# SilasK/drep

Measured on AMD Instinct MI355X. Metric: genome pairs/sec (mash dist, k=21 s=1000) + sketch GB/s, at 1/2/4/8 GPUs, higher is better.
Workload: dtype u64; 1 GPU; 1000 synthetic 5000000 bp genomes, k=21, s=1000 (BASELINE.json configs[1]); step = sketch + all-pairs (one GPU: no all-gather); genomes=1000, genome_bp=5000000, k=21, sketch=1000, family_size=100, parallelism=sketch: genome shards; all-pairs: balanced row shards; RCCL all-gather

## Files before the change

drep_amd/_lib.py:

```python
from __future__ import annotations

import ctypes as C
import importlib.util
import os
import sys
import threading
from typing import Optional, Sequence, Tuple

import numpy as np

_HERE = os.path.dirname(os.path.abspath(__file__))
LIB_PATH = os.environ.get("DREPHIP_LIB", os.path.join(_HERE, "lib", "libdrephip.so"))

ERR = {0: "OK", -1: "invalid argument", -2: "HIP error", -3: "I/O error", -4: "out of memory",
       -5: "unsupported", -6: "internal error"}


class DrepHipError(RuntimeError):
    pass


_lib = None
_lock = threading.Lock()

u64p = np.ctypeslib.ndpointer(dtype=np.uint64, flags="C_CONTIGUOUS")
u32p = np.ctypeslib.ndpointer(dtype=np.uint32, flags="C_CONTIGUOUS")
u16p = np.ctypeslib.ndpointer(dtype=np.uint16, flags="C_CONTIGUOUS")
u8p = np.ctypeslib.ndpointer(dtype=np.uint8, flags="C_CONTIGUOUS")
f64p = np.ctypeslib.ndpointer(dtype=np.float64, flags="C_CONTIGUOUS")
vp = C.c_void_p

SIGNATURES = {
    "drephip_version": (C.c_int, []),
    "drephip_build_id": (C.c_char_p, []),
    "drephip_last_error": (C.c_char_p, []),
    "drephip_device_count": (C.c_int, [C.POINTER(C.c_int)]),
    "drephip_create": (C.c_int, [C.c_int, C.c_int, C.c_uint32, C.c_uint32, C.POINTER(vp)]),
    "drephip_destroy": (C.c_int, [vp]),
    "drephip_max_sketch": (C.c_uint32, []),
    "drephip_tile_bases": (C.c_uint64, []),
    "drephip_padded_bases": (C.c_uint64, [u64p, C.c_uint32]),
    "drephip_fasta_info": (C.c_int, [C.c_char_p, C.c_int, C.POINTER(C.c_uint64), C.POINTER(C.c_uint64),
                                     C.POINTER(C.c_uint32), C.POINTER(C.c_uint64)]),
    "drephip_fasta_pack": (C.c_int, [C.c_char_p, C.c_int, u32p, u32p, C.c_uint64, C.c_uint64,
                                     C.POINTER(C.c_uint64), C.POINTER(C.c_uint64)]),
    "drephip_sketch": (C.c_int, [vp, u8p, u64p, C.c_uint32, u64p, C.c_uint32, u64p, u32p, u64p]),
    "drephip_sketch_files": (C.c_int, [vp, C.POINTER(C.c_char_p), C.c_uint32, C.c_int, u64p, u32p, u64p]),
    "drephip_last_ingest_stats": (C.c_int, [vp, C.POINTER(C.c_double), C.POINTER(C.c_double),
                                            C.POINTER(C.c_double), C.POINTER(C.c_uint32)]),
    "drephip_last_ingest_phases": (C.c_int, [vp, C.POINTER(C.c_double), C.POINTER(C.c_double),
                                             C.POINTER(C.c_uint32)]),
    "drephip_sketch_device": (C.c_int, [vp, vp, vp, u64p, u64p, u64p, C.c_uint32, vp, vp, vp]),
    "drephip_sketch_device_async": (C.c_int, [vp, vp, vp, u64p, u64p, u64p, C.c_uint32, vp, vp, vp]),
    "drephip_sketch_wait": (C.c_int, [vp, C.POINTER(C.c_int)]),
    "drephip_synth_device": (C.c_int, [vp, C.c_uint64, C.c_uint32, C.c_uint32, C.c_uint32, C.c_uint64,
                                       vp, vp, vp]),
    "drephip_prefilter_eval": (C.c_int, [u64p, u64p, C.c_uint64, C.c_uint64, u8p, u8p]),
    "drephip_allpairs": (C.c_int, [vp, u64p, u32p, C.c_uint32, u16p, vp]),
    "drephip_allpairs_rows": (C.c_int, [vp, u64p, u32p, C.c_uint32, C.c_uint32, C.c_uint32, vp, vp]),
    "drephip_allpairs_device": (C.c_int, [vp, vp, vp, C.c_uint32, C.c_uint32, C.c_uint32, vp, vp, vp]),
    "drephip_allpairs_device_async": (C.c_int, [vp, vp, vp, C.c_uint32, C.c_uint32, C.c_uint32, vp, vp, vp]),
    "drephip_allpairs_wait": (C.c_int, [vp]),
    "drephip_screen_geometry": (C.c_int, [vp, C.POINTER(C.c_uint32)]),
    "drephip_screen_part": (C.c_int, [vp, vp, vp, C.c_uint32, C.c_uint32, C.c_uint32, C.POINTER(C.c_uint64),
                                      C.POINTER(C.c_uint32), C.POINTER(C.c_uint32), vp]),
    "drephip_screen_part_copy": (C.c_int, [vp, vp, vp, vp]),
    "drephip_screen_worth": (C.c_int, [vp, C.c_uint32, C.c_uint64, C.POINTER(C.c_int), C.POINTER(C.c_int)]),
    "drephip_allpairs_device_marked": (C.c_int, [vp, vp, vp, C.c_uint32, C.c_uint32, C.c_uint32, vp, vp, vp,
                                                 C.c_uint64, vp, C.c_uint64, vp]),
    "drephip_allpairs_merge_device": (C.c_int, [vp, vp, vp, C.c_uint32, C.c_uint32, C.c_uint32, vp, vp, vp]),
    "drephip_allpairs_sparse_device": (C.c_int, [vp, vp, vp, C.c_uint32, C.c_uint32, C.c_uint32, vp, C.c_uint64,
                                                 C.POINTER(C.c_uint64), vp]),
    "drephip_allpairs_sparse": (C.c_int, [vp, u64p, u32p, C.c_uint32, C.c_uint32, C.c_uint32, vp, C.c_uint64,
                                          C.POINTER(C.c_uint64)]),
    "drephip_last_sparse_stats": (C.c_int, [vp, C.POINTER(C.c_uint32), C.POINTER(C.c_uint64), C.POINTER(C.c_uint64),
                                            C.POINTER(C.c_uint64)]),
    "drephip_distance_lut": (C.c_int, [C.c_int, C.c_uint32, f64p]),
    "drephip_write_mash_table": (C.c_int, [C.c_char_p, C.POINTER(C.c_char_p), C.c_uint32, vp, vp, C.c_uint32,
                                           vp, vp, u16p, f64p, C.c_int]),
    "drephip_set_allpairs_path": (C.c_int, [vp, C.c_int, C.c_uint32]),
    "drephip_linkage": (C.c_int, [vp, f64p, C.c_uint32, C.c_int, f64p]),
    "drephip_linkage_counts_device": (C.c_int, [vp, vp, vp, C.c_uint32, u32p, f64p, C.c_uint32,
                                                np.ctypeslib.ndpointer(dtype=np.int32, flags="C_CONTIGUOUS"),
                                                C.c_int, f64p, vp]),
    "drephip_linkage_square": (C.c_int, [vp, np.ctypeslib.ndpointer(dtype=np.float32, flags="C_CONTIGUOUS"),
                                         C.c_uint32, C.c_int, f64p]),
    "drephip_mdb_square": (C.c_int, [C.c_uint32, vp, vp, C.c_uint32, vp, C.c_uint32, vp, vp, C.c_int, vp, vp, vp,
                                     vp, C.c_int]),
    "drephip_pivot_scan": (C.c_int, [C.c_uint64, vp, vp, C.c_int, C.c_uint32, u8p, u8p, C.POINTER(C.c_uint64),
                                     C.c_int]),
    "drephip_pivot_fill": (C.c_int, [C.c_uint64, vp, vp, C.c_int, vp, vp, C.c_uint32, vp, C.c_uint32, C.c_uint32,
                                     C.c_uint64, vp, C.c_int]),
    "drephip_linkage_reserve": (C.c_int, [vp, C.c_uint32]),
    "drephip_set_linkage_path": (C.c_int, [vp, C.c_int]),
    "drephip_linkage_sparse": (C.c_int, [C.c_uint32, C.c_uint64, u32p, u32p, f64p, C.c_int, f64p]),
    "drephip_last_linkage_info": (C.c_int, [vp, C.POINTER(C.c_int), C.POINTER(C.c_uint64), C.POINTER(C.c_uint32),
                                            C.POINTER(C.c_uint32)]),
    "drephip_last_linkage_stats": (C.c_int, [vp] + [C.POINTER(C.c_double)] * 5),
    "drephip_last_linkage_launches": (C.c_int, [vp, C.POINTER(C.c_uint64)]),
    "drephip_set_timing": (C.c_int, [vp, C.c_int]),
    "drephip_last_kernel_ms": (C.c_int, [vp, C.c_int, C.POINTER(C.c_double), C.POINTER(C.c_int)]),
    "drephip_set_allpairs_screen": (C.c_int, [vp, C.c_int]),
    "drephip_last_screen_stats": (C.c_int, [vp, C.POINTER(C.c_int), C.POINTER(C.c_uint64), C.POINTER(C.c_uint64),
                                             C.POINTER(C.c_uint64), C.POINTER(C.c_uint64), C.POINTER(C.c_uint64)]),
}


def _preload_torch_hip_runtime() -> None:
    if "torch" in sys.modules:
        return
# ... 52 lines not shown
    return hashlib.sha256(listing.encode()).hexdigest()


def build_id() -> dict:
    raw = lib().drephip_build_id().decode()
    return dict(kv.split("=", 1) for kv in raw.split(";") if "=" in kv)


def check(rc: int, what: str) -> None:
    if rc != 0:
        msg = lib().drephip_last_error().decode("utf-8", "replace")
        raise DrepHipError("%s failed (%s): %s" % (what, ERR.get(rc, rc), msg))


def device_count() -> int:
    n = C.c_int(0)
    rc = lib().drephip_device_count(C.byref(n))
    return n.value if rc == 0 else 0


def max_sketch() -> int:
    return int(lib().drephip_max_sketch())


def tile_bases() -> int:
    return int(lib().drephip_tile_bases())


def padded_bases(rec_len: Sequence[int]) -> int:
    a = np.ascontiguousarray(rec_len, dtype=np.uint64)
    return int(lib().drephip_padded_bases(a if len(a) else np.zeros(1, np.uint64), len(a)))


def distance_lut(denom: int, k: int = 21) -> np.ndarray:
    out = np.zeros(denom + 1, dtype=np.float64)
    check(lib().drephip_distance_lut(k, denom, out), "drephip_distance_lut")
    return out


def prefilter_eval(q1: np.ndarray, q2: np.ndarray, T: int) -> Tuple[np.ndarray, np.ndarray]:
    q1 = np.ascontiguousarray(q1, dtype=np.uint64)
    q2 = np.ascontiguousarray(q2, dtype=np.uint64)
    if q1.shape != q2.shape or q1.ndim != 1:
        raise ValueError("q1 and q2 must be equal-length vectors")
    n = len(q1)
    ok = np.zeros(max(n, 1), np.uint8)
    exact = np.zeros(max(n, 1), np.uint8)
    z = np.zeros(1, np.uint64)
    check(lib().drephip_prefilter_eval(q1 if n else z, q2 if n else z, n, int(T), ok, exact),
          "drephip_prefilter_eval")
    return ok[:n].astype(bool), exact[:n].astype(bool)


def write_mash_table(path: str, names: Sequence[str], common: np.ndarray, denom: Optional[np.ndarray], s: int,
                     dist: np.ndarray, pval: np.ndarray, self_count: np.ndarray, self_pval: np.ndarray,
                     threads: int = 0) -> None:
    N = len(names)
    npairs = N * (N - 1) // 2
    common = np.ascontiguousarray(common, dtype=np.uint16)
    dist = np.ascontiguousarray(dist, dtype=np.float64)
    pval = np.ascontiguousarray(pval, dtype=np.float64)
    for a in (common, dist, pval) + ((denom,) if denom is not None else ()):
        if len(a) != npairs:
            raise ValueError("condensed arrays must hold N(N-1)/2 = %d entries" % npairs)
    den = None if denom is None else np.ascontiguousarray(denom, dtype=np.uint16)
    arr = (C.c_char_p * max(N, 1))(*[os.fsencode(n) for n in names])
    check(lib().drephip_write_mash_table(os.fsencode(path), arr, N, common.ctypes.data,
                                         None if den is None else den.ctypes.data, int(s), dist.ctypes.data,
                                         pval.ctypes.data, np.ascontiguousarray(self_count, dtype=np.uint16),
                                         np.ascontiguousarray(self_pval, dtype=np.float64), int(threads)),
          "drephip_write_mash_table(%s)" % path)


def fasta_info(path: str, k: int = 21):
    length = C.c_uint64(0)
    padded = C.c_uint64(0)
    nrec = C.c_uint32(0)
    nk = C.c_uint64(0)
    check(lib().drephip_fasta_info(path.encode(), k, C.byref(length), C.byref(padded), C.byref(nrec),
                                   C.byref(nk)), "drephip_fasta_info(%s)" % path)
    return {"length": length.value, "padded": padded.value, "n_records": nrec.value, "n_kmers": nk.value}


def _ptr(a: Optional[np.ndarray]):
    return None if a is None else a.ctypes.data


def mdb_square(N: int, common: np.ndarray, denom: Optional[np.ndarray], s: int, lut32: np.ndarray,
               lut_off: np.ndarray, codes: np.ndarray, threads: int = 0, want_sim: bool = True):
    common = np.ascontiguousarray(common, dtype=np.uint16)
    den = None if denom is None else np.ascontiguousarray(denom, dtype=np.uint16)
    lut32 = np.ascontiguousarray(lut32, dtype=np.float32)
    lut_off = np.ascontiguousarray(lut_off, dtype=np.int32)
    codes = np.ascontiguousarray(codes)
    if codes.dtype not in (np.int8, np.int16, np.int32) or len(codes) != N or len(lut_off) != s + 1:
        raise ValueError("codes must be N int8/int16/int32 category codes and lut_off s+1 offsets")
    npairs = N * (N - 1) // 2
    if len(common) != npairs or (den is not None and len(den) != npairs):
        raise ValueError("condensed arrays must hold N(N-1)/2 = %d entries" % npairs)
    codes32 = codes.astype(np.int32)
    g1 = np.empty(N * N, dtype=codes.dtype)
    g2 = np.empty(N * N, dtype=codes.dtype)
    dist = np.empty(N * N, dtype=np.float32)
    sim = np.empty(N * N, dtype=np.float32) if want_sim else None
    check(lib().drephip_mdb_square(N, _ptr(common) if npairs else None, _ptr(den) if npairs else None, int(s),
                                   _ptr(lut32), len(lut32), _ptr(lut_off), _ptr(codes32), codes.dtype.itemsize,
# ... 376 lines not shown
```

drep_amd/csrc/api.cpp:

```cpp
#include "ctx.h"
#include "prefilter.h"
#include "../../include/drephip.h"

#include <algorithm>
#include <atomic>
#include <chrono>
#include <cmath>
#include <condition_variable>
#include <mutex>
#include <cstdlib>
#include <cstring>
#include <new>
#include <thread>
#include <vector>

#define DREPHIP_EXPORT extern "C" __attribute__((visibility("default")))

namespace drephip {

static thread_local std::string g_err;
void set_error(const std::string &msg) { g_err = msg; }

int scratch(drephip_ctx *ctx, const char *name, size_t bytes, void **out) {
    DevBuf &b = ctx->bufs[name];
    if (bytes == 0) bytes = 8;
    if (b.bytes < bytes) {
        const size_t want = std::max(bytes, b.bytes + b.bytes / 4);
        if (b.ptr) {
            HIPC(hipStreamSynchronize(ctx->stream));
            HIPC(hipDeviceSynchronize());
            HIPC(hipFree(b.ptr));
            b.ptr = nullptr; b.bytes = 0;
        }
        ctx->alloc_gen++;
        hipError_t e = hipMalloc(&b.ptr, want);
        if (e != hipSuccess) {
            set_error(std::string("hipMalloc(") + std::to_string(want) + ") for " + name + ": " +
                      hipGetErrorString(e));
            b.ptr = nullptr;
            return DREPHIP_ERR_NOMEM;
        }
        b.bytes = want;
    }
    *out = b.ptr;
    return DREPHIP_OK;
}

int pinned_host(drephip_ctx *ctx, const char *name, size_t bytes, void **out) {
    DevBuf &b = ctx->pinned[name];
    if (bytes == 0) bytes = 8;
    if (b.bytes < bytes) {
        if (b.ptr) {
            HIPC(hipStreamSynchronize(ctx->stream));
// ... 818 lines not shown
    int rc;
    if ((rc = scratch(ctx, "ap_in_h", (uint64_t)N * s * 8, (void **)&d_h))) return rc;
    if ((rc = scratch(ctx, "ap_in_n", N * 4ull, (void **)&d_n))) return rc;
    if (cap && (rc = scratch(ctx, "sp_out", cap * 16, (void **)&d_p))) return rc;
    HIPC(hipMemcpyAsync(d_h, hashes, (uint64_t)N * s * 8, hipMemcpyHostToDevice, st));
    HIPC(hipMemcpyAsync(d_n, nhash, N * 4ull, hipMemcpyHostToDevice, st));
    timing_begin(ctx);
    rc = allpairs_sparse_impl(ctx, d_h, d_n, N, row0, row1, (uint4 *)d_p, cap, n_pairs, st);
    if (rc && rc != DREPHIP_ERR_NOMEM) return rc;
    timing_collect(ctx);
    const uint64_t have = std::min(*n_pairs, cap);
    if (have) HIPC(hipMemcpyAsync(pairs, d_p, have * 16, hipMemcpyDeviceToHost, st));
    HIPC(hipStreamSynchronize(st));
    return rc;
}

DREPHIP_EXPORT int drephip_last_sparse_stats(drephip_ctx *ctx, uint32_t *blocks, uint64_t *direct, uint64_t *fallback,
                                             uint64_t *scratch_bytes) {
    if (!ctx) { set_error("null context"); return DREPHIP_ERR_ARG; }
    if (blocks) *blocks = ctx->sparse.blocks;
    if (direct) *direct = ctx->sparse.direct;
    if (fallback) *fallback = ctx->sparse.fallback;
    if (scratch_bytes) *scratch_bytes = ctx->sparse.scratch_bytes;
    return DREPHIP_OK;
}

DREPHIP_EXPORT int drephip_distance_lut(int k, uint32_t denom, double *lut) {
    if (!lut || k < 1 || denom == 0) { set_error("bad argument"); return DREPHIP_ERR_ARG; }
    for (uint32_t c = 0; c <= denom; c++) {
        double d;
        if (c == denom) d = 0.0;
        else if (c == 0) d = 1.0;
        else {
            const double j = (double)c / (double)denom;
            d = -std::log(2.0 * j / (1.0 + j)) / (double)k;
            if (d > 1.0) d = 1.0;
        }
        lut[c] = d;
    }
    return DREPHIP_OK;
}

DREPHIP_EXPORT int drephip_prefilter_eval(const uint64_t *q1, const uint64_t *q2, uint64_t n, uint64_t T,
                                          uint8_t *pass, uint8_t *exact) {
    if (n && (!q1 || !q2 || !pass || !exact)) { set_error("bad argument"); return DREPHIP_ERR_ARG; }
    const uint32_t Tp = prefilter_bound(T);
    for (uint64_t i = 0; i < n; i++) {
        pass[i] = prefilter_hi(q1[i], q2[i]) <= Tp;
        exact[i] = murmur_fin(q1[i], q2[i]) <= T;
    }
    return DREPHIP_OK;
}

constexpr uint64_t kSparseMaxCells = 1ull << 31;
constexpr uint64_t kSparseMaxPairs = 1ull << 26;

static uint64_t env_u64(const char *name, uint64_t dflt) {
    if (const char *e = std::getenv(name)) return std::strtoull(e, nullptr, 10);
    return dflt;
}
static uint64_t sparse_cells(const drephip_ctx *ctx) {
    return ctx->link_path == DREPHIP_LINK_PATH_SPARSE ? kSparseMaxCells : env_u64("DREPHIP_LINK_SPARSE_CELLS", 1ull << 28);
}
static uint32_t sparse_maxcomp(const drephip_ctx *ctx) {
    return ctx->link_path == DREPHIP_LINK_PATH_SPARSE ? 0xFFFFFFFFu
                                                      : (uint32_t)env_u64("DREPHIP_LINK_SPARSE_MAXCOMP", 4096);
}
static uint64_t sparse_pair_cap(const drephip_ctx *ctx, uint32_t n) {
    const uint64_t all = (uint64_t)n * (n - 1) / 2;
    const uint64_t cap = ctx->link_path == DREPHIP_LINK_PATH_SPARSE ? kSparseMaxPairs
                                                                    : std::min<uint64_t>(kSparseMaxPairs, 32ull * n + (1ull << 20));
    return std::min(all, cap);
}

DREPHIP_EXPORT int drephip_set_linkage_path(drephip_ctx *ctx, int path) {
    GUARD_CTX(ctx);
    if (path < DREPHIP_LINK_PATH_AUTO || path > DREPHIP_LINK_PATH_SPARSE) { set_error("bad linkage path"); return DREPHIP_ERR_ARG; }
    ctx->link_path = path;
    return DREPHIP_OK;
}

DREPHIP_EXPORT int drephip_linkage_sparse(uint32_t n, uint64_t npairs, const uint32_t *i, const uint32_t *j,
                                          const double *v, int method, double *Z) {
    if (n < 2) return DREPHIP_OK;
    if (!Z || (npairs && (!i || !j || !v))) { set_error("null argument"); return DREPHIP_ERR_ARG; }
    return linkage_sparse_impl(n, npairs, i, j, v, method, kSparseMaxCells, 0xFFFFFFFFu, Z, nullptr, 1);
}

static int linkage_condensed_sparse(drephip_ctx *ctx, const double *y, uint32_t n, int method, double *Z, int *rc) {
    *rc = DREPHIP_OK;
    if (ctx->link_path == DREPHIP_LINK_PATH_DENSE) return 0;
    const double t0 = std::chrono::duration<double>(std::chrono::steady_clock::now().time_since_epoch()).count();
    const uint64_t np_all = (uint64_t)n * (n - 1) / 2, cap = sparse_pair_cap(ctx, n);
    const unsigned T = host_threads();
    std::vector<uint32_t> rb(T + 1, n - 1);
    rb[0] = 0;
    for (unsigned k = 1; k < T; k++) {
        const uint64_t target = np_all * k / T;
        uint32_t lo = rb[k - 1], hi = n - 1;
        while (lo < hi) {
            const uint32_t mid = lo + (hi - lo) / 2;
            if ((uint64_t)mid * n - (uint64_t)mid * (mid + 1) / 2 < target) lo = mid + 1; else hi = mid;
        }
        rb[k] = lo;
    }
    std::vector<std::vector<uint32_t>> qi(T), qj(T);
// ... 208 lines not shown
```

drep_amd/csrc/prefilter.h:

```cpp
#pragma once

#include <hip/hip_runtime.h>
#include <stdint.h>

namespace drephip {

constexpr uint64_t kFmixC1 = 0xff51afd7ed558ccdULL;
constexpr uint64_t kFmixC2 = 0xc4ceb9fe1a85ec53ULL;

__host__ __device__ __forceinline__ uint32_t mulhi32(uint32_t a, uint32_t b) {
#if defined(__HIP_DEVICE_COMPILE__)
    return __umulhi(a, b);
#else
    return (uint32_t)(((uint64_t)a * b) >> 32);
#endif
}

__host__ __device__ __forceinline__ uint64_t fmix64_q(uint64_t k) {
    k ^= k >> 33; k *= kFmixC1;
    k ^= k >> 33;
    return k;
}
__host__ __device__ __forceinline__ uint64_t fmix_mul(uint64_t q) { return q * kFmixC2; }
__host__ __device__ __forceinline__ uint64_t murmur_fin(uint64_t q1, uint64_t q2) {
    const uint64_t p1 = fmix_mul(q1), p2 = fmix_mul(q2);
    return (p1 ^ (p1 >> 33)) + (p2 ^ (p2 >> 33));
}

__host__ __device__ __forceinline__ uint32_t prefilter_bound(uint64_t T) {
    return __builtin_elementwise_add_sat((uint32_t)(T >> 32), 2u);
}
__host__ __device__ __forceinline__ uint32_t prefilter_hi(uint64_t q1, uint64_t q2) {
    const uint64_t Q = q1 + q2;
    const uint32_t a = (uint32_t)Q, b = (uint32_t)(Q >> 32);
    return mulhi32(a, (uint32_t)kFmixC2) + a * (uint32_t)(kFmixC2 >> 32) + b * (uint32_t)kFmixC2 + 1u;
}

}
```

drep_amd/csrc/sketch.hip:

```cpp

#include "ctx.h"
#include "prefilter.h"
#include "../../include/drephip.h"

#include <algorithm>
#include <cstddef>
#include <cstdio>
#include <cstdlib>
#include <cstring>
#include <vector>

namespace drephip {

__device__ __forceinline__ void set_insert(unsigned long long *S, uint32_t mask, uint32_t *cnt,
                                           uint32_t limit, uint64_t h) {
    if (__hip_atomic_load(cnt, __ATOMIC_RELAXED, __HIP_MEMORY_SCOPE_AGENT) >= limit) return;
    uint32_t slot = (uint32_t)h & mask;
    for (uint32_t probe = 0; probe <= mask; probe++) {
        unsigned long long old = atomicCAS(&S[slot], (unsigned long long)kEmpty, (unsigned long long)h);
        if (old == kEmpty) { atomicAdd(cnt, 1u); return; }
        if (old == h) return;
        slot = (slot + 1) & mask;
    }
}

__device__ __forceinline__ uint64_t rotl64_ab(uint64_t x, int r) {
    const uint32_t lo = (uint32_t)x, hi = (uint32_t)(x >> 32);
    uint32_t nlo, nhi;
    if (r < 32) {
        nhi = __builtin_amdgcn_alignbit(hi, lo, 32 - r);
        nlo = __builtin_amdgcn_alignbit(lo, hi, 32 - r);
    } else {
        nhi = __builtin_amdgcn_alignbit(lo, hi, 64 - r);
        nlo = __builtin_amdgcn_alignbit(hi, lo, 64 - r);
    }
    return ((uint64_t)nhi << 32) | nlo;
}
__device__ __forceinline__ uint64_t x5_plus(uint64_t x, uint64_t c) {
    uint64_t y;
    asm("v_lshl_add_u64 %0, %1, 2, %1" : "=v"(y) : "v"(x));
    return y + c;
}
__device__ __forceinline__ uint64_t add64(uint64_t a, uint64_t b) {
    uint64_t y;
    asm("v_lshl_add_u64 %0, %1, 0, %2" : "=v"(y) : "v"(a), "v"(b));
    return y;
}
#ifndef DREPHIP_SK_STAGE
#define DREPHIP_SK_STAGE 128
#endif
constexpr uint32_t kStage = DREPHIP_SK_STAGE;

typedef uint32_t u32x4 __attribute__((ext_vector_type(4)));
typedef uint32_t u32x2 __attribute__((ext_vector_type(2)));
struct SketchTablesQ {
    u32x4 e1[256];
    u32x4 e2[256];
    u32x2 b1[256];
    u32x2 b2[256];
    uint64_t t3[1024];
};

__device__ __forceinline__ uint32_t ascii4(uint32_t x) {
    const uint32_t sel = ((x >> 6) & 3u) | (((x >> 4) & 3u) << 8) | (((x >> 2) & 3u) << 16) | ((x & 3u) << 24);
    return __builtin_amdgcn_perm(0u, 0x54474341u, sel);
}

__device__ void build_tables(SketchTablesQ &tb, uint32_t tid, uint32_t nthreads) {
    constexpr uint64_t c1 = 0x87c37b91114253d5ULL, c2 = 0x4cf5ad432745937fULL;
    for (uint32_t x = tid; x < 256; x += nthreads) {
        const uint32_t a = ascii4(x);
        const uint64_t A1 = (uint64_t)a * c1, A2 = (uint64_t)a * c2;
        const uint32_t x1 = (uint32_t)A1, x2 = (uint32_t)A2;
        const uint32_t ta1 = (uint32_t)(A1 >> 32), ta2 = (uint32_t)(A2 >> 32);
        const uint64_t t1 = ((uint64_t)x1 << 31) * c2 + ((uint64_t)(ta1 << 31) << 32);
        const uint64_t t2 = ((uint64_t)(x2 & 0x7fffffffu) << 33) * c1 + (uint64_t)(x2 >> 31) * c1;
        tb.e1[x] = u32x4{(uint32_t)t1, (uint32_t)(t1 >> 32), ta1, 0u};
        constexpr uint32_t d1hi = (uint32_t)((c1 * 2) >> 32);
        tb.e2[x] = u32x4{(uint32_t)t2, (uint32_t)(t2 >> 32), ta2, ta2 * d1hi};
        const uint32_t m1 = a * (uint32_t)c1;
        tb.b1[x] = u32x2{m1, m1 << 31};
        const uint32_t m2 = a * (uint32_t)c2;
        tb.b2[x] = u32x2{m2, m2 * d1hi};
    }
    for (uint32_t y = tid; y < 1024; y += nthreads) {
        const uint64_t k3 = (uint64_t)ascii4(y >> 2) | ((uint64_t)ascii4((y & 3u) << 6) & 0xffu) << 32;
        tb.t3[y] = (rotl64_ab(k3 * c1, 31) * c2) ^ 21u;
    }
}

constexpr uint32_t kTabVec = sizeof(SketchTablesQ) / 16;
constexpr uint32_t kSketchTabShifts = 4u | (3u << 8);
static_assert(sizeof(SketchTablesQ) % 16 == 0, "table image is copied in 16-byte pieces");
__global__ __launch_bounds__(256) void k_sketch_tables(SketchTablesQ *__restrict__ img) {
    __shared__ SketchTablesQ tb;
    build_tables(tb, threadIdx.x, 256);
    __syncthreads();
    const u32x4 *src = (const u32x4 *)&tb;
    u32x4 *dst = (u32x4 *)img;
    for (uint32_t i = threadIdx.x; i < kTabVec; i += 256) dst[i] = src[i];
}

__device__ __forceinline__ uint32_t rev_fields16(uint32_t x) {
    const uint32_t y = __builtin_bitreverse32(x);
    return ((y >> 1) & 0x55555555u) | ((y & 0x55555555u) << 1);
}

__device__ __forceinline__ uint64_t mad64(uint32_t a, uint32_t b, uint64_t c) {
    return (uint64_t)a * b + c;
}

struct MEnt { u32x4 e1; u32x2 f1; u32x4 e2; u32x2 f2; uint64_t k3; };
#ifndef DREPHIP_SK_ABLATE
#define DREPHIP_SK_ABLATE 0
#endif
__device__ __forceinline__ MEnt fetch_ent(const SketchTablesQ &tb, uint32_t hi, uint32_t lo, uint32_t sh) {
    const char *base = (const char *)&tb;
#if DREPHIP_SK_ABLATE
    const uint32_t s16 = sh & 0xfu, s8 = (sh >> 8) & 0xfu, km = (sh >> 16) & 0x3ffu;
#if DREPHIP_SK_ABLATE == 2
    (void)base; (void)s16; (void)s8; (void)km;
    return MEnt{u32x4{hi, lo, hi, lo}, u32x2{lo, hi}, u32x4{lo, hi, lo, hi}, u32x2{hi, lo},
                ((uint64_t)hi << 32) | lo};
#endif
    return MEnt{*(const u32x4 *)(base + (((hi >> 24) & km) << s16)),
                *(const u32x2 *)(base + offsetof(SketchTablesQ, b1) + (((hi >> 16) & km & 0xffu) << s8)),
                *(const u32x4 *)(base + offsetof(SketchTablesQ, e2) + (((hi >> 8) & km & 0xffu) << s16)),
                *(const u32x2 *)(base + offsetof(SketchTablesQ, b2) + ((hi & km & 0xffu) << s8)),
                tb.t3[(lo >> 22) & km]};
#else
    const uint32_t s16 = sh & 0xffu, s8 = sh >> 8;
    return MEnt{*(const u32x4 *)(base + ((hi >> 24) << s16)),
                *(const u32x2 *)(base + offsetof(SketchTablesQ, b1) + (((hi >> 16) & 0xffu) << s8)),
                *(const u32x4 *)(base + offsetof(SketchTablesQ, e2) + (((hi >> 8) & 0xffu) << s16)),
                *(const u32x2 *)(base + offsetof(SketchTablesQ, b2) + ((hi & 0xffu) << s8)),
                tb.t3[lo >> 22]};
#endif
}
__device__ __forceinline__ void murmur21_ent(const MEnt &E, uint32_t seed, uint64_t &q1, uint64_t &q2) {
    constexpr uint64_t c1 = 0x87c37b91114253d5ULL, c2 = 0x4cf5ad432745937fULL;
    constexpr uint64_t d1 = c1 * 2;
    const u32x4 e1 = E.e1;
    const u32x2 f1 = E.f1;
    const u32x4 e2 = E.e2;
    const u32x2 f2 = E.f2;
    const uint64_t k3 = E.k3;
    const uint32_t X1 = e1.z + f1.x;
    const uint32_t X2 = e2.z + f2.x;
    const uint64_t tt1 = ((uint64_t)e1.y << 32) | e1.x;
    const uint64_t tt2 = ((uint64_t)e2.y << 32) | e2.x;
    const uint32_t h = X1 >> 1;
    const uint64_t P1 = mad64(h, (uint32_t)c2, tt1);
    const uint32_t g1hi = (uint32_t)(P1 >> 32) + h * (uint32_t)(c2 >> 32) + f1.y;
    uint64_t h1 = ((uint64_t)g1hi << 32) | ((uint32_t)P1 ^ seed);
    h1 = x5_plus(rotl64_ab(h1, 27), 5ull * seed + 0x52dce729);
    const uint64_t P2 = mad64(X2, (uint32_t)d1, tt2);
    const uint32_t g2hi = (uint32_t)(P2 >> 32) + e2.w + f2.y;
    uint64_t h2 = ((uint64_t)g2hi << 32) | ((uint32_t)P2 ^ seed);
    h2 = x5_plus(add64(rotl64_ab(h2, 31), h1), 0x38495ab5);
    h1 ^= k3;
    h2 ^= 21u;
    h1 = add64(h1, h2);
    h2 = add64(h2, h1);
    q1 = fmix64_q(h1);
    q2 = fmix64_q(h2);
}
__device__ __forceinline__ void murmur21_q(const SketchTablesQ &tb, uint32_t hi, uint32_t lo, uint32_t seed,
                                           uint32_t sh, uint64_t &q1, uint64_t &q2) {
    murmur21_ent(fetch_ent(tb, hi, lo, sh), seed, q1, q2);
}
#ifndef DREPHIP_SK_BATCH
#define DREPHIP_SK_BATCH 2
#endif
#ifndef DREPHIP_SK_MINW
#define DREPHIP_SK_MINW 1
#endif
constexpr uint32_t kHashLane = 64;
template <int LANE, int BATCH>
__global__ __launch_bounds__(kTile / LANE, DREPHIP_SK_MINW) void k_sketch_hash21(
    const SketchTablesQ *__restrict__ img, const uint32_t *__restrict__ codes, const uint32_t *__restrict__ valid,
    const uint64_t *__restrict__ tile_base, const uint32_t *__restrict__ tile_genome,
    const uint64_t *__restrict__ thr, unsigned long long *__restrict__ sets,
    uint32_t *__restrict__ cnt, uint32_t set_log2, uint32_t limit, uint32_t seed, uint64_t wlast, uint32_t sh) {
    constexpr uint32_t WG = kTile / LANE;
    constexpr int NCH = LANE / 16;
    __shared__ SketchTablesQ tb;
    __shared__ uint64_t stage[kStage];
    __shared__ uint32_t nstage;
    const uint32_t t = blockIdx.x;
    const uint32_t g = tile_genome[t];
    const uint64_t T = thr[g];
    const uint32_t Tp = prefilter_bound(T);
    const uint64_t start = tile_base[t] + (uint64_t)threadIdx.x * LANE;
    const uint32_t mask = (1u << set_log2) - 1;
    unsigned long long *S = sets + ((uint64_t)g << set_log2);
    uint32_t *C = cnt + g;
    if (threadIdx.x == 0) nstage = 0;
    {
        const u32x4 *src = (const u32x4 *)img;
        u32x4 *dst = (u32x4 *)&tb;
        for (uint32_t i = threadIdx.x; i < kTabVec; i += WG) dst[i] = src[i];
    }

    const uint64_t w0 = tile_base[t] / 16 - 2;
    const uint64_t nrec = (wlast + 1 - w0) * 4;
    const __amdgpu_buffer_rsrc_t crs = __builtin_amdgcn_make_buffer_rsrc(
        (void *)(codes + w0), (short)0, (int)(nrec < 0xFFFFFFF0ull ? nrec : 0xFFFFFFF0ull), 0x00020000);
    const uint32_t lane_off = threadIdx.x * (LANE / 16) * 4;
    auto ld = [&](int j) -> uint32_t {
        return __builtin_amdgcn_raw_buffer_load_b32(crs, lane_off, (uint32_t)__builtin_amdgcn_readfirstlane(j + 2) * 4u, 0);
    };
    uint32_t nf0 = ~ld(-2), nf1 = ~ld(-1), nf2 = ~ld(0);
    uint32_t r0 = rev_fields16(~nf0), r1 = rev_fields16(~nf1), r2 = rev_fields16(~nf2);
    uint32_t f3 = ld(1);
    uint32_t r3 = rev_fields16(f3);
    uint32_t fnext = ld(2);
    const uint32_t *vw = valid + (start - kWarm) / 32;
    uint64_t vhist = (uint64_t)vw[0] << 32;
    uint32_t vcur = vw[1];
    __syncthreads();

    static_assert(NCH == 4, "unroll count");
#pragma unroll 4
    for (int wi = 0; wi < NCH; wi++) {
        const uint32_t vbits = (vcur >> ((wi & 1) * 16)) & 0xffffu;
        if (wi + 1 < NCH && (wi & 1)) vcur = vw[2 + (wi >> 1)];
        vhist = (vhist >> 16) | ((uint64_t)vbits << 48);
        auto canon = [&](int r) -> uint64_t {
            uint32_t chi, clo, fhi, flo;
            if (r == 15) { chi = nf2; clo = nf1; }
            else {
                chi = __builtin_amdgcn_alignbit(nf2, nf1, 2 * (r + 1));
                clo = __builtin_amdgcn_alignbit(nf1, nf0, 2 * (r + 1));
            }
            if (r < 4) {
                fhi = __builtin_amdgcn_alignbit(r0, r1, 32 - 2 * (r + 12));
                flo = __builtin_amdgcn_alignbit(r1, r2, 32 - 2 * (r + 12));
            } else if (r == 4) {
                fhi = r1; flo = r2;
            } else {
                fhi = __builtin_amdgcn_alignbit(r1, r2, 32 - 2 * (r - 4));
                flo = __builtin_amdgcn_alignbit(r2, r3, 32 - 2 * (r - 4));
            }
            const uint64_t fw = ((uint64_t)fhi << 32) | flo;
            const uint64_t rc = ((uint64_t)chi << 32) | clo;
            return fw <= rc ? fw : rc;
        };
#pragma unroll
        for (int b0 = 0; b0 < 16; b0 += BATCH) {
            uint64_t p1[BATCH], p2[BATCH];
            bool hit = false;
#pragma unroll
            for (int b = 0; b < BATCH; b++) {
                const uint64_t cc = canon(b0 + b);
                murmur21_q(tb, (uint32_t)(cc >> 32), (uint32_t)cc, seed, sh, p1[b], p2[b]);
                hit |= prefilter_hi(p1[b], p2[b]) <= Tp;
            }
            if (__builtin_expect(hit, 0)) {
#pragma unroll
                for (int b = 0; b < BATCH; b++) {
                    const uint64_t h = murmur_fin(p1[b], p2[b]);
                    const bool ok = (~(uint32_t)(vhist >> (28 + b0 + b)) & 0x1FFFFFu) == 0;
                    if (h <= T && ok) {
                        const uint32_t slot = atomicAdd(&nstage, 1u);
                        if (slot < kStage) stage[slot] = h;
                        else set_insert(S, mask, C, limit, h);
                    }
                }
            }
        }
        nf0 = nf1; nf1 = nf2; nf2 = ~f3;
        r0 = r1; r1 = r2; r2 = r3;
        f3 = fnext;
        r3 = rev_fields16(f3);
        fnext = ld(wi + 3);
    }
    __syncthreads();
    const uint32_t n = min(nstage, kStage);
    for (uint32_t i = threadIdx.x; i < n; i += WG) set_insert(S, mask, C, limit, stage[i]);
}

enum : uint8_t { ST_OK = 0, ST_UP = 1, ST_DOWN = 2 };

__device__ __forceinline__ void finalize_reset(unsigned long long *S, uint32_t slots, uint32_t *cnt_g) {
    for (uint32_t i = threadIdx.x; i < slots; i += blockDim.x) S[i] = kEmpty;
    __syncthreads();
    if (threadIdx.x == 0) *cnt_g = 0;
}

template <int MAXC, int NB>
__global__ __launch_bounds__(1024) void k_sketch_finalize_bucket(
    unsigned long long *__restrict__ sets, uint32_t *__restrict__ cnt,
    const uint64_t *__restrict__ thr, const uint32_t *__restrict__ glist, uint32_t set_log2,
    uint32_t maxc, uint32_t s, uint64_t *__restrict__ out, uint32_t *__restrict__ nhash,
    uint8_t *__restrict__ status) {
    constexpr uint32_t WG = 1024, PER = NB / WG, LOGNB = __builtin_ctz(NB);
    static_assert(NB % WG == 0 && (NB & (NB - 1)) == 0, "NB: power of two, multiple of the workgroup");
    __shared__ uint64_t buf[MAXC];
    __shared__ uint32_t bk[NB];
    __shared__ uint32_t wsum[WG / 64];
    const uint32_t g = glist[blockIdx.x];
    const uint32_t n = cnt[g];
    const uint32_t tid = threadIdx.x;
    const uint64_t T = thr[g];
    unsigned long long *S = sets + ((uint64_t)g << set_log2);
    const uint32_t slots = 1u << set_log2;
    if (n > maxc || (n < s && T < kMaxThr)) {
        if (tid == 0) status[g] = n > maxc ? ST_DOWN : ST_UP;
        finalize_reset(S, slots, cnt + g);
        return;
    }
    const uint32_t tbits = 64 - __builtin_clzll(T | 1);
    const uint32_t shift = tbits > LOGNB ? tbits - LOGNB : 0;
    for (uint32_t i = tid; i < NB; i += WG) bk[i] = 0;
    __syncthreads();
    if (tid == 0) cnt[g] = 0;
    for (uint32_t i = tid; i < slots; i += WG) {
        const uint64_t v = S[i];
        if (v != kEmpty) atomicAdd(&bk[min((uint32_t)(v >> shift), (uint32_t)NB - 1u)], 1u);
    }
    __syncthreads();
    uint32_t loc[PER], sum = 0;
#pragma unroll
    for (int j = 0; j < PER; j++) { loc[j] = sum; sum += bk[tid * PER + j]; }
    uint32_t inc = sum;
#pragma unroll
    for (int d = 1; d < 64; d <<= 1) {
        const uint32_t y = __shfl_up(inc, d, 64);
        if ((tid & 63) >= d) inc += y;
    }
    if ((tid & 63) == 63) wsum[tid >> 6] = inc;
    __syncthreads();
// ... 407 lines not shown
```

include/drephip.h:

```cpp
#ifndef DREPHIP_H
#define DREPHIP_H

#include <stdint.h>

#ifdef __cplusplus
extern "C" {
#endif

#define DREPHIP_OK               0
#define DREPHIP_ERR_ARG         -1
#define DREPHIP_ERR_HIP         -2
#define DREPHIP_ERR_IO          -3
#define DREPHIP_ERR_NOMEM       -4
#define DREPHIP_ERR_UNSUPPORTED -5
#define DREPHIP_ERR_INTERNAL    -6

typedef struct drephip_ctx drephip_ctx;

int drephip_version(void);

const char *drephip_build_id(void);

const char *drephip_last_error(void);

int drephip_device_count(int *n);

int drephip_create(int device, int k, uint32_t s, uint32_t seed, drephip_ctx **out);
int drephip_destroy(drephip_ctx *ctx);

uint32_t drephip_max_sketch(void);

uint64_t drephip_tile_bases(void);

uint64_t drephip_padded_bases(const uint64_t *rec_len, uint32_t n_rec);

int drephip_fasta_info(const char *path, int k, uint64_t *length, uint64_t *padded,
                       uint32_t *n_records, uint64_t *n_kmers);

int drephip_fasta_pack(const char *path, int k, uint32_t *codes, uint32_t *valid,
                       uint64_t base_off, uint64_t cap_bases, uint64_t *length,
                       uint64_t *n_kmers);

int drephip_sketch(drephip_ctx *ctx, const uint8_t *seq, const uint64_t *rec_off, uint32_t n_rec,
                   const uint64_t *genome_rec_off, uint32_t n_genomes,
                   uint64_t *hashes_out, uint32_t *nhash_out, uint64_t *length_out);

int drephip_sketch_files(drephip_ctx *ctx, const char *const *paths, uint32_t n_genomes,
                         int threads, uint64_t *hashes_out, uint32_t *nhash_out,
                         uint64_t *length_out);

int drephip_last_ingest_stats(drephip_ctx *ctx, double *produce_s, double *gpu_s, double *wall_s,
                              uint32_t *batches);

int drephip_last_ingest_phases(drephip_ctx *ctx, double *read_thread_s, double *pack_thread_s,
                               uint32_t *overflow);

int drephip_sketch_device(drephip_ctx *ctx, const uint32_t *d_codes, const uint32_t *d_valid,
                          const uint64_t *h_base_off, const uint64_t *h_padded,
                          const uint64_t *h_nkmers, uint32_t n_genomes,
                          uint64_t *d_hashes, uint32_t *d_nhash, void *stream);

int drephip_sketch_device_async(drephip_ctx *ctx, const uint32_t *d_codes, const uint32_t *d_valid,
                                const uint64_t *h_base_off, const uint64_t *h_padded,
                                const uint64_t *h_nkmers, uint32_t n_genomes,
                                uint64_t *d_hashes, uint32_t *d_nhash, void *stream);

int drephip_sketch_wait(drephip_ctx *ctx, int *redone);

int drephip_synth_device(drephip_ctx *ctx, uint64_t seed, uint32_t g0, uint32_t n,
                         uint32_t family_size, uint64_t L, uint32_t *d_codes, uint32_t *d_valid,
                         void *stream);

int drephip_prefilter_eval(const uint64_t *q1, const uint64_t *q2, uint64_t n, uint64_t T,
                           uint8_t *pass, uint8_t *exact);

int drephip_allpairs(drephip_ctx *ctx, const uint64_t *hashes, const uint32_t *nhash, uint32_t N,
                     uint16_t *common_out, uint16_t *denom_out );

int drephip_allpairs_rows(drephip_ctx *ctx, const uint64_t *hashes, const uint32_t *nhash, uint32_t N,
                          uint32_t row0, uint32_t row1, uint16_t *common_out, uint16_t *denom_out );

int drephip_allpairs_device(drephip_ctx *ctx, const uint64_t *d_hashes, const uint32_t *d_nhash,
                            uint32_t N, uint32_t row0, uint32_t row1, uint16_t *d_common,
                            uint16_t *d_denom, void *stream);

int drephip_allpairs_device_async(drephip_ctx *ctx, const uint64_t *d_hashes, const uint32_t *d_nhash,
                                  uint32_t N, uint32_t row0, uint32_t row1, uint16_t *d_common,
                                  uint16_t *d_denom, void *stream);
int drephip_allpairs_wait(drephip_ctx *ctx);

int drephip_allpairs_merge_device(drephip_ctx *ctx, const uint64_t *d_hashes, const uint32_t *d_nhash,
                                  uint32_t N, uint32_t row0, uint32_t row1, uint16_t *d_common,
                                  uint16_t *d_denom, void *stream);

int drephip_distance_lut(int k, uint32_t denom, double *lut );

int drephip_write_mash_table(const char *path, const char *const *names, uint32_t N,
                             const uint16_t *common, const uint16_t *denom , uint32_t s,
                             const double *dist, const double *pval, const uint16_t *self_count,
                             const double *self_pval, int threads);

#define DREPHIP_AP_AUTO 0
#define DREPHIP_AP_TABLE 1
#define DREPHIP_AP_BAND 2
#define DREPHIP_AP_MERGE 3
int drephip_set_allpairs_path(drephip_ctx *ctx, int path, uint32_t band_cap);

#define DREPHIP_SCREEN_AUTO 0
#define DREPHIP_SCREEN_ON 1
#define DREPHIP_SCREEN_OFF 2
int drephip_set_allpairs_screen(drephip_ctx *ctx, int mode);
int drephip_last_screen_stats(drephip_ctx *ctx, int *used, uint64_t *entries, uint64_t *runs, uint64_t *checks,
                              uint64_t *marked, uint64_t *simple);

int drephip_screen_geometry(drephip_ctx *ctx, uint32_t *rows_per_tile);
int drephip_screen_part(drephip_ctx *ctx, const uint64_t *d_hashes, const uint32_t *d_nhash, uint32_t N,
                        uint32_t part, uint32_t nparts, uint64_t *checks, uint32_t *n_cells, uint32_t *n_records,
                        void *stream);
int drephip_screen_part_copy(drephip_ctx *ctx, uint32_t *d_cells, uint32_t *d_records, void *stream);
int drephip_screen_worth(drephip_ctx *ctx, uint32_t N, uint64_t checks, int *applies , int *use);
int drephip_allpairs_device_marked(drephip_ctx *ctx, const uint64_t *d_hashes, const uint32_t *d_nhash, uint32_t N,
                                   uint32_t row0, uint32_t row1, uint16_t *d_common, uint16_t *d_denom,
                                   const uint32_t *d_cells, uint64_t n_cells, const uint32_t *d_records,
                                   uint64_t n_records, void *stream);

int drephip_allpairs_sparse_device(drephip_ctx *ctx, const uint64_t *d_hashes, const uint32_t *d_nhash,
                                   uint32_t N, uint32_t row0, uint32_t row1,
// ... 55 lines not shown
```

Baseline: 65.70 million genome pairs/s.

## Slim canonical k-mer selection and defer final hash to staged insert

Canonical k-mer selection now compares only the high word plus a 3-bit tail offset, skipping the full 64-bit lo word construction, and the t3 table lookup indexes by that precomputed byte offset. The hot loop stages raw (q1,q2) pairs that pass the prefilter and runs the final murmur and threshold check only during the staged insert, which takes the full hash off the hit path. fmix64 multiplication is split into explicit 32-bit pieces. Staging doubles shared-memory stage size, and the canonical tie-breaking now relies on the high word alone. A host-side canon_eval entry is added for testing.

```diff
diff --git a/drep_amd/_lib.py b/drep_amd/_lib.py
--- a/drep_amd/_lib.py
+++ b/drep_amd/_lib.py
@@ -56,6 +56,7 @@
     "drephip_synth_device": (C.c_int, [vp, C.c_uint64, C.c_uint32, C.c_uint32, C.c_uint32, C.c_uint64,
                                        vp, vp, vp]),
     "drephip_prefilter_eval": (C.c_int, [u64p, u64p, C.c_uint64, C.c_uint64, u8p, u8p]),
+    "drephip_canon_eval": (C.c_int, [u32p, C.c_uint64, C.c_uint32, u32p, u32p]),
     "drephip_allpairs": (C.c_int, [vp, u64p, u32p, C.c_uint32, u16p, vp]),
     "drephip_allpairs_rows": (C.c_int, [vp, u64p, u32p, C.c_uint32, C.c_uint32, C.c_uint32, vp, vp]),
     "drephip_allpairs_device": (C.c_int, [vp, vp, vp, C.c_uint32, C.c_uint32, C.c_uint32, vp, vp, vp]),
@@ -214,6 +215,18 @@
     return ok[:n].astype(bool), exact[:n].astype(bool)
 
 
+def canon_eval(words: np.ndarray, r: int) -> Tuple[np.ndarray, np.ndarray]:
+    words = np.ascontiguousarray(words, dtype=np.uint32)
+    if words.ndim != 2 or words.shape[1] != 3:
+        raise ValueError("words must be n x 3")
+    n = len(words)
+    hi = np.zeros(max(n, 1), np.uint32)
+    tail = np.zeros(max(n, 1), np.uint32)
+    check(lib().drephip_canon_eval(words if n else np.zeros((1, 3), np.uint32), n, int(r), hi, tail),
+          "drephip_canon_eval")
+    return hi[:n], tail[:n]
+
+
 def write_mash_table(path: str, names: Sequence[str], common: np.ndarray, denom: Optional[np.ndarray], s: int,
                      dist: np.ndarray, pval: np.ndarray, self_count: np.ndarray, self_pval: np.ndarray,
                      threads: int = 0) -> None:
diff --git a/drep_amd/csrc/api.cpp b/drep_amd/csrc/api.cpp
--- a/drep_amd/csrc/api.cpp
+++ b/drep_amd/csrc/api.cpp
@@ -1,4 +1,5 @@
 #include "ctx.h"
+#include "canon.h"
 #include "prefilter.h"
 #include "../../include/drephip.h"
 
@@ -923,6 +924,17 @@
     return DREPHIP_OK;
 }
 
+DREPHIP_EXPORT int drephip_canon_eval(const uint32_t *words, uint64_t n, uint32_t r, uint32_t *hi, uint32_t *tail) {
+    if (r > 15 || (n && (!words || !hi || !tail))) { set_error("bad argument"); return DREPHIP_ERR_ARG; }
+    for (uint64_t i = 0; i < n; i++) {
+        const uint32_t *f = words + 3 * i;
+        uint32_t toff;
+        canon_cut(~f[0], ~f[1], ~f[2], rev_fields16(f[0]), rev_fields16(f[1]), rev_fields16(f[2]), (int)r, hi[i], toff);
+        tail[i] = toff >> 3;
+    }
+    return DREPHIP_OK;
+}
+
 constexpr uint64_t kSparseMaxCells = 1ull << 31;
 constexpr uint64_t kSparseMaxPairs = 1ull << 26;
 
diff --git a/drep_amd/csrc/canon.h b/drep_amd/csrc/canon.h
--- /dev/null
+++ b/drep_amd/csrc/canon.h
@@ -0,0 +1,43 @@
+#pragma once
+
+#include <hip/hip_runtime.h>
+#include <stdint.h>
+
+namespace drephip {
+
+__host__ __device__ __forceinline__ uint32_t alignbit32(uint32_t hi, uint32_t lo, uint32_t s) {
+#if defined(__HIP_DEVICE_COMPILE__)
+    return __builtin_amdgcn_alignbit(hi, lo, s);
+#else
+    return (uint32_t)((((uint64_t)hi << 32) | lo) >> (s & 31u));
+#endif
+}
+
+__host__ __device__ __forceinline__ uint32_t rev_fields16(uint32_t x) {
+    const uint32_t y = __builtin_bitreverse32(x);
+    return ((y >> 1) & 0x55555555u) | ((y & 0x55555555u) << 1);
+}
+
+constexpr uint32_t kTailOffMask = 0x1FF8u;
+
+__host__ __device__ __forceinline__ uint32_t field_to_3(uint32_t x, int at) {
+    return at >= 3 ? x >> (at - 3) : x << (3 - at);
+}
+
+__host__ __device__ __forceinline__ void canon_cut(uint32_t nf0, uint32_t nf1, uint32_t nf2, uint32_t r0,
+                                                   uint32_t r1, uint32_t r2, int r, uint32_t &hi, uint32_t &toff) {
+    const uint32_t chi = r == 15 ? nf2 : alignbit32(nf2, nf1, 2 * (r + 1));
+    const uint32_t fhi = r < 4 ? alignbit32(r0, r1, 32 - 2 * (r + 12)) : r == 4 ? r1 : alignbit32(r1, r2, 32 - 2 * (r - 4));
+    uint32_t ft, ct;
+    if (r < 4) {
+        ft = alignbit32(r1, r2, 27 - 2 * r);
+        ct = alignbit32(nf1, nf0, 21 + 2 * r);
+    } else {
+        ft = field_to_3(r2, 30 - 2 * r);
+        ct = field_to_3(nf1, 2 * (r - 4));
+    }
+    hi = fhi < chi ? fhi : chi;
+    toff = (fhi < chi ? ft : ct) & kTailOffMask;
+}
+
+}
diff --git a/drep_amd/csrc/prefilter.h b/drep_amd/csrc/prefilter.h
--- a/drep_amd/csrc/prefilter.h
+++ b/drep_amd/csrc/prefilter.h
@@ -17,7 +17,11 @@
 }
 
 __host__ __device__ __forceinline__ uint64_t fmix64_q(uint64_t k) {
-    k ^= k >> 33; k *= kFmixC1;
+    k ^= k >> 33;
+    const uint32_t lo = (uint32_t)k, hi = (uint32_t)(k >> 32);
+    const uint32_t t = hi * (uint32_t)kFmixC1;
+    const uint32_t cross = (uint32_t)((uint64_t)lo * (uint32_t)(kFmixC1 >> 32) + t);
+    k = (uint64_t)lo * (uint32_t)kFmixC1 + ((uint64_t)cross << 32);
     k ^= k >> 33;
     return k;
 }
diff --git a/drep_amd/csrc/sketch.hip b/drep_amd/csrc/sketch.hip
--- a/drep_amd/csrc/sketch.hip
+++ b/drep_amd/csrc/sketch.hip
@@ -1,4 +1,5 @@
 
+#include "canon.h"
 #include "ctx.h"
 #include "prefilter.h"
 #include "../../include/drephip.h"
@@ -53,6 +54,7 @@
 
 typedef uint32_t u32x4 __attribute__((ext_vector_type(4)));
 typedef uint32_t u32x2 __attribute__((ext_vector_type(2)));
+typedef uint64_t u64x2 __attribute__((ext_vector_type(2)));
 struct SketchTablesQ {
     u32x4 e1[256];
     u32x4 e2[256];
@@ -101,11 +103,6 @@
     for (uint32_t i = threadIdx.x; i < kTabVec; i += 256) dst[i] = src[i];
 }
 
-__device__ __forceinline__ uint32_t rev_fields16(uint32_t x) {
-    const uint32_t y = __builtin_bitreverse32(x);
-    return ((y >> 1) & 0x55555555u) | ((y & 0x55555555u) << 1);
-}
-
 __device__ __forceinline__ uint64_t mad64(uint32_t a, uint32_t b, uint64_t c) {
     return (uint64_t)a * b + c;
 }
@@ -114,27 +111,27 @@
 #ifndef DREPHIP_SK_ABLATE
 #define DREPHIP_SK_ABLATE 0
 #endif
-__device__ __forceinline__ MEnt fetch_ent(const SketchTablesQ &tb, uint32_t hi, uint32_t lo, uint32_t sh) {
+__device__ __forceinline__ MEnt fetch_ent(const SketchTablesQ &tb, uint32_t hi, uint32_t toff, uint32_t sh) {
     const char *base = (const char *)&tb;
 #if DREPHIP_SK_ABLATE
     const uint32_t s16 = sh & 0xfu, s8 = (sh >> 8) & 0xfu, km = (sh >> 16) & 0x3ffu;
 #if DREPHIP_SK_ABLATE == 2
     (void)base; (void)s16; (void)s8; (void)km;
-    return MEnt{u32x4{hi, lo, hi, lo}, u32x2{lo, hi}, u32x4{lo, hi, lo, hi}, u32x2{hi, lo},
-                ((uint64_t)hi << 32) | lo};
+    return MEnt{u32x4{hi, toff, hi, toff}, u32x2{toff, hi}, u32x4{toff, hi, toff, hi}, u32x2{hi, toff},
+                ((uint64_t)hi << 32) | toff};
 #endif
     return MEnt{*(const u32x4 *)(base + (((hi >> 24) & km) << s16)),
                 *(const u32x2 *)(base + offsetof(SketchTablesQ, b1) + (((hi >> 16) & km & 0xffu) << s8)),
                 *(const u32x4 *)(base + offsetof(SketchTablesQ, e2) + (((hi >> 8) & km & 0xffu) << s16)),
                 *(const u32x2 *)(base + offsetof(SketchTablesQ, b2) + ((hi & km & 0xffu) << s8)),
-                tb.t3[(lo >> 22) & km]};
+                *(const uint64_t *)(base + offsetof(SketchTablesQ, t3) + (toff & (km << 3)))};
 #else
     const uint32_t s16 = sh & 0xffu, s8 = sh >> 8;
     return MEnt{*(const u32x4 *)(base + ((hi >> 24) << s16)),
                 *(const u32x2 *)(base + offsetof(SketchTablesQ, b1) + (((hi >> 16) & 0xffu) << s8)),
                 *(const u32x4 *)(base + offsetof(SketchTablesQ, e2) + (((hi >> 8) & 0xffu) << s16)),
                 *(const u32x2 *)(base + offsetof(SketchTablesQ, b2) + ((hi & 0xffu) << s8)),
-                tb.t3[lo >> 22]};
+                *(const uint64_t *)(base + offsetof(SketchTablesQ, t3) + toff)};
 #endif
 }
 __device__ __forceinline__ void murmur21_ent(const MEnt &E, uint32_t seed, uint64_t &q1, uint64_t &q2) {
@@ -165,9 +162,9 @@
     q1 = fmix64_q(h1);
     q2 = fmix64_q(h2);
 }
-__device__ __forceinline__ void murmur21_q(const SketchTablesQ &tb, uint32_t hi, uint32_t lo, uint32_t seed,
+__device__ __forceinline__ void murmur21_q(const SketchTablesQ &tb, uint32_t hi, uint32_t toff, uint32_t seed,
                                            uint32_t sh, uint64_t &q1, uint64_t &q2) {
-    murmur21_ent(fetch_ent(tb, hi, lo, sh), seed, q1, q2);
+    murmur21_ent(fetch_ent(tb, hi, toff, sh), seed, q1, q2);
 }
 #ifndef DREPHIP_SK_BATCH
 #define DREPHIP_SK_BATCH 2
@@ -185,7 +182,7 @@
     constexpr uint32_t WG = kTile / LANE;
     constexpr int NCH = LANE / 16;
     __shared__ SketchTablesQ tb;
-    __shared__ uint64_t stage[kStage];
+    __shared__ u64x2 stage[kStage];
     __shared__ uint32_t nstage;
     const uint32_t t = blockIdx.x;
     const uint32_t g = tile_genome[t];
@@ -226,45 +223,30 @@
         const uint32_t vbits = (vcur >> ((wi & 1) * 16)) & 0xffffu;
         if (wi + 1 < NCH && (wi & 1)) vcur = vw[2 + (wi >> 1)];
         vhist = (vhist >> 16) | ((uint64_t)vbits << 48);
-        auto canon = [&](int r) -> uint64_t {
-            uint32_t chi, clo, fhi, flo;
-            if (r == 15) { chi = nf2; clo = nf1; }
-            else {
-                chi = __builtin_amdgcn_alignbit(nf2, nf1, 2 * (r + 1));
-                clo = __builtin_amdgcn_alignbit(nf1, nf0, 2 * (r + 1));
-            }
-            if (r < 4) {
-                fhi = __builtin_amdgcn_alignbit(r0, r1, 32 - 2 * (r + 12));
-                flo = __builtin_amdgcn_alignbit(r1, r2, 32 - 2 * (r + 12));
-            } else if (r == 4) {
-                fhi = r1; flo = r2;
-            } else {
-                fhi = __builtin_amdgcn_alignbit(r1, r2, 32 - 2 * (r - 4));
-                flo = __builtin_amdgcn_alignbit(r2, r3, 32 - 2 * (r - 4));
-            }
-            const uint64_t fw = ((uint64_t)fhi << 32) | flo;
-            const uint64_t rc = ((uint64_t)chi << 32) | clo;
-            return fw <= rc ? fw : rc;
-        };
+        auto canon = [&](int r, uint32_t &hi, uint32_t &toff) { canon_cut(nf0, nf1, nf2, r0, r1, r2, r, hi, toff); };
 #pragma unroll
         for (int b0 = 0; b0 < 16; b0 += BATCH) {
             uint64_t p1[BATCH], p2[BATCH];
-            bool hit = false;
+            bool pf[BATCH], hit = false;
 #pragma unroll
             for (int b = 0; b < BATCH; b++) {
-                const uint64_t cc = canon(b0 + b);
-                murmur21_q(tb, (uint32_t)(cc >> 32), (uint32_t)cc, seed, sh, p1[b], p2[b]);
-                hit |= prefilter_hi(p1[b], p2[b]) <= Tp;
+                uint32_t chw, toff;
+                canon(b0 + b, chw, toff);
+                murmur21_q(tb, chw, toff, seed, sh, p1[b], p2[b]);
+                pf[b] = prefilter_hi(p1[b], p2[b]) <= Tp;
+                hit |= pf[b];
             }
             if (__builtin_expect(hit, 0)) {
 #pragma unroll
                 for (int b = 0; b < BATCH; b++) {
-                    const uint64_t h = murmur_fin(p1[b], p2[b]);
                     const bool ok = (~(uint32_t)(vhist >> (28 + b0 + b)) & 0x1FFFFFu) == 0;
-                    if (h <= T && ok) {
+                    if (pf[b] && ok) {
                         const uint32_t slot = atomicAdd(&nstage, 1u);
-                        if (slot < kStage) stage[slot] = h;
-                        else set_insert(S, mask, C, limit, h);
+                        if (slot < kStage) stage[slot] = u64x2{p1[b], p2[b]};
+                        else {
+                            const uint64_t h = murmur_fin(p1[b], p2[b]);
+                            if (h <= T) set_insert(S, mask, C, limit, h);
+                        }
                     }
                 }
             }
@@ -277,7 +259,11 @@
     }
     __syncthreads();
     const uint32_t n = min(nstage, kStage);
-    for (uint32_t i = threadIdx.x; i < n; i += WG) set_insert(S, mask, C, limit, stage[i]);
+    for (uint32_t i = threadIdx.x; i < n; i += WG) {
+        const u64x2 q = stage[i];
+        const uint64_t h = murmur_fin(q.x, q.y);
+        if (h <= T) set_insert(S, mask, C, limit, h);
+    }
 }
 
 enum : uint8_t { ST_OK = 0, ST_UP = 1, ST_DOWN = 2 };
diff --git a/include/drephip.h b/include/drephip.h
--- a/include/drephip.h
+++ b/include/drephip.h
@@ -73,6 +73,8 @@
 
 int drephip_prefilter_eval(const uint64_t *q1, const uint64_t *q2, uint64_t n, uint64_t T,
                            uint8_t *pass, uint8_t *exact);
+
+int drephip_canon_eval(const uint32_t *words, uint64_t n, uint32_t r, uint32_t *hi, uint32_t *tail);
 
 int drephip_allpairs(drephip_ctx *ctx, const uint64_t *hashes, const uint32_t *nhash, uint32_t N,
                      uint16_t *common_out, uint16_t *denom_out );
```

Measured after the change: 67.87 million genome pairs/s (median of 6 runs). 3.3% higher.
